# DAIRLab/dair_pll

Measured on NVIDIA B200. Metric: ContactNets loss+backward samples/s, cube fp64, higher is better.
Workload: dtype f64

## Files before the change

dair_pll_b200/csrc/cn_cube.cuh:

```cuda
#pragma once
#include "cn_common.cuh"

#ifndef CN_STAT_LS
#define CN_STAT_LS()
#define CN_STAT_UNIT()
#endif

namespace cn {

constexpr int CUBE_NQ = 7, CUBE_NV = 6, CUBE_NX = 13, CUBE_NC = 4, CUBE_K = 12;
constexpr int CUBE_NPARAM = 14;
constexpr int CUBE_PROB_FIELDS = 33;

template <typename T> struct CubeParams {
  T m, c[3], Isym[6];
  T mu;
  T h[3];
  T dt, eps, inv_eps, grav;
  T Io[6];
  T Isym_inv[6];
  T inv_m;
  T dscale[6];
};

template <typename T>
CN_HD void cube_params_init(CubeParams<T>& P, const T* inertia, const T* mu, const T* half, T dt, T eps) {
  P.m = inertia[0];
  for (int i = 0; i < 3; ++i) P.c[i] = inertia[1 + i];
  for (int i = 0; i < 6; ++i) P.Isym[i] = inertia[4 + i];
  P.mu = mu[0];
  for (int i = 0; i < 3; ++i) P.h[i] = half[i];
  P.dt = dt; P.eps = eps; P.inv_eps = T(1) / eps; P.grav = T(9.81);
  const T cx = P.c[0], cy = P.c[1], cz = P.c[2], m = P.m;
  P.Io[0] = P.Isym[0] + m * (cy * cy + cz * cz);
  P.Io[1] = P.Isym[1] + m * (cx * cx + cz * cz);
  P.Io[2] = P.Isym[2] + m * (cx * cx + cy * cy);
  P.Io[3] = P.Isym[3] - m * cx * cy;
  P.Io[4] = P.Isym[4] - m * cx * cz;
  P.Io[5] = P.Isym[5] - m * cy * cz;
  sym3_inv(P.Isym, P.Isym_inv);
  P.inv_m = T(1) / m;
  P.dscale[0] = T(1) / P.Io[0]; P.dscale[1] = T(1) / P.Io[1]; P.dscale[2] = T(1) / P.Io[2];
  P.dscale[3] = P.dscale[4] = P.dscale[5] = P.inv_m;
}

template <typename T> struct CubeProb {
  T* p;
  int s;
  CN_HD T& IW(int i) const { return p[i * s]; }
  CN_HD T& mcW(int i) const { return p[(6 + i) * s]; }
  CN_HD T& rho(int k) const { return p[(9 + k) * s]; }
  CN_HD T& q(int k) const { return p[(21 + k) * s]; }
};

template <typename T>
CN_HD void cube_minv(const CubeParams<T>& P, const T* R, const T* tau, const T* frc, T* aw, T* av) {
  T fb[3], cxf[3], rhs[3], cxa[3], rc[3];
  rot3t(R, frc, fb);
  cross3(P.c, fb, cxf);
  for (int i = 0; i < 3; ++i) rhs[i] = tau[i] - cxf[i];
  sym3_mul(P.Isym_inv, rhs, aw);
  cross3(P.c, aw, cxa);
  rot3(R, cxa, rc);
  for (int i = 0; i < 3; ++i) av[i] = frc[i] * P.inv_m + rc[i];
}

template <typename T>
CN_HD void cube_mass_mul(const CubeParams<T>& P, const CubeProb<T>& S, const T* u, T* o) {
  const T I0 = S.IW(0), I1 = S.IW(1), I2 = S.IW(2), I3 = S.IW(3), I4 = S.IW(4), I5 = S.IW(5);
  const T mc[3] = {S.mcW(0), S.mcW(1), S.mcW(2)};
  T b[3], c[3];
  cross3(mc, u + 3, b);
  cross3(mc, u, c);
  o[0] = I0 * u[0] + I3 * u[1] + I4 * u[2] + b[0];
  o[1] = I3 * u[0] + I1 * u[1] + I5 * u[2] + b[1];
  o[2] = I4 * u[0] + I5 * u[1] + I2 * u[2] + b[2];
  for (int i = 0; i < 3; ++i) o[3 + i] = P.m * u[3 + i] - c[i];
}

template <typename T> CN_HD uint32_t cube_select_corners(const T* d, const T* h) {
  const T a0 = t_abs(d[0]) * h[0], a1 = t_abs(d[1]) * h[1], a2 = t_abs(d[2]) * h[2];
  const uint32_t best = (d[0] >= T(0) ? 4u : 0u) | (d[1] >= T(0) ? 2u : 0u) | (d[2] >= T(0) ? 1u : 0u);
  const bool c01 = a0 <= a1, c12 = a1 <= a2, c02 = a0 <= a2;
  const int is = c01 ? (c02 ? 0 : 2) : (c12 ? 1 : 2);
  const int il = c01 ? (c12 ? 2 : 1) : (c02 ? 2 : 0);
  const int im = 3 - is - il;
  const T lo01 = t_min(a0, a1), hi01 = t_max(a0, a1);
  const T as = t_min(lo01, a2), al = t_max(hi01, a2), am = t_max(lo01, t_min(hi01, a2));
  const uint32_t bs = 4u >> is, bm = 4u >> im, bl = 4u >> il;
  const uint32_t v3 = (as + am <= al) ? (best ^ bs ^ bm) : (best ^ bl);
  uint32_t mask = (1u << best) | (1u << (best ^ bs)) | (1u << (best ^ bm)) | (1u << v3);
  uint32_t sel = 0;
#pragma unroll
  for (int c = 0; c < 4; ++c) {
#if defined(__CUDA_ARCH__)
    const uint32_t i = (uint32_t)(__ffs((int)mask) - 1);
#else
    const uint32_t i = (uint32_t)(__builtin_ffs((int)mask) - 1);
#endif
    mask &= mask - 1u;
    sel |= i << (3 * c);
  }
  return sel;
}

template <typename T> CN_HD T sgn_bit(uint32_t sel, int c, int axis) {
  return ((sel >> (3 * c + 2 - axis)) & 1u) ? T(1) : T(-1);
}

template <typename T, int UNR>
CN_HD void cube_geometry(const CubeParams<T>& P, const T* quat, T* R, uint32_t& sel, const CubeProb<T>& S) {
  quat_to_rot(quat, R);
  T A[9];
#pragma unroll
  for (int i = 0; i < 3; ++i) {
    const T r0 = R[3 * i], r1 = R[3 * i + 1], r2 = R[3 * i + 2];
    A[3 * i + 0] = r0 * P.Io[0] + r1 * P.Io[3] + r2 * P.Io[4];
    A[3 * i + 1] = r0 * P.Io[3] + r1 * P.Io[1] + r2 * P.Io[5];
    A[3 * i + 2] = r0 * P.Io[4] + r1 * P.Io[5] + r2 * P.Io[2];
  }
  S.IW(0) = A[0] * R[0] + A[1] * R[1] + A[2] * R[2];
  S.IW(1) = A[3] * R[3] + A[4] * R[4] + A[5] * R[5];
  S.IW(2) = A[6] * R[6] + A[7] * R[7] + A[8] * R[8];
  S.IW(3) = A[0] * R[3] + A[1] * R[4] + A[2] * R[5];
  S.IW(4) = A[0] * R[6] + A[1] * R[7] + A[2] * R[8];
  S.IW(5) = A[3] * R[6] + A[4] * R[7] + A[5] * R[8];
  T cW[3];
  rot3(R, P.c, cW);
#pragma unroll
  for (int i = 0; i < 3; ++i) S.mcW(i) = P.m * cW[i];
  const T d[3] = {-R[6], -R[7], -R[8]};
  sel = cube_select_corners(d, P.h);
  T Rh[9];
#pragma unroll
  for (int i = 0; i < 3; ++i)
#pragma unroll
    for (int k = 0; k < 3; ++k) Rh[3 * i + k] = R[3 * i + k] * P.h[k];
#pragma unroll UNR
  for (int c = 0; c < CUBE_NC; ++c) {
    const T sx = sgn_bit<T>(sel, c, 0), sy = sgn_bit<T>(sel, c, 1), sz = sgn_bit<T>(sel, c, 2);
#pragma unroll
    for (int i = 0; i < 3; ++i) S.rho(3 * c + i) = sx * Rh[3 * i] + sy * Rh[3 * i + 1] + sz * Rh[3 * i + 2];
  }
}

template <typename T>
CN_HD void cube_free_accel(const CubeParams<T>& P, const T* R, const T* wB, T* aw, T* av) {
  T Iw[3], wIw[3], gB[3], cg[3], tau[3], wc[3], wwc[3], Rwwc[3], frc[3];
  sym3_mul(P.Io, wB, Iw);
  cross3(wB, Iw, wIw);
  gB[0] = -P.grav * R[6]; gB[1] = -P.grav * R[7]; gB[2] = -P.grav * R[8];
  cross3(P.c, gB, cg);
  for (int i = 0; i < 3; ++i) tau[i] = -wIw[i] + P.m * cg[i];
  cross3(wB, P.c, wc);
  cross3(wB, wc, wwc);
  rot3(R, wwc, Rwwc);
  for (int i = 0; i < 3; ++i) frc[i] = -P.m * Rwwc[i];
  frc[2] -= P.m * P.grav;
  cube_minv(P, R, tau, frc, aw, av);
}

template <typename T>
CN_HD void cube_contact_residual(const CubeParams<T>& P, const CubeProb<T>& S, int c, const T* u, T* rho, T* r) {
  rho[0] = S.rho(3 * c); rho[1] = S.rho(3 * c + 1); rho[2] = S.rho(3 * c + 2);
  T e[3];
  cross3_add(u, rho, u + 3, e);
  r[0] = P.mu * e[0] + S.q(3 * c);
  r[1] = P.mu * e[1] + S.q(3 * c + 1);
  r[2] = e[2] + S.q(3 * c + 2);
}

template <typename T, bool WANT_H, int UNR>
CN_HD void cube_eval(const CubeParams<T>& P, const CubeProb<T>& S, const T* u, T* g, T* H, T& res2, T& scale2) {
  T Mu[6];
  cube_mass_mul(P, S, u, Mu);
  T z[6] = {T(0), T(0), T(0), T(0), T(0), T(0)};
  if (WANT_H) {
    const T m0 = S.mcW(0), m1 = S.mcW(1), m2 = S.mcW(2);
    H[0] = S.IW(0); H[7] = S.IW(1); H[14] = S.IW(2);
    H[6] = S.IW(3); H[12] = S.IW(4); H[13] = S.IW(5);
    H[18] = T(0); H[19] = m2;   H[20] = -m1;
    H[24] = -m2;  H[25] = T(0); H[26] = m0;
    H[30] = m1;   H[31] = -m0;  H[32] = T(0);
    H[21] = P.m; H[28] = P.m; H[35] = P.m; H[27] = T(0); H[33] = T(0); H[34] = T(0);
  }
#pragma unroll UNR
  for (int c = 0; c < CUBE_NC; ++c) {
    T rho[3], r[3], f[3], K[6];
    cube_contact_residual(P, S, c, u, rho, r);
    cone_eval<T, WANT_H>(r, P.inv_eps, P.mu, f, K);
    const T ft[3] = {P.mu * f[0], P.mu * f[1], f[2]};
    cross3_add(rho, ft, z, z);
#pragma unroll
    for (int i = 0; i < 3; ++i) z[3 + i] += ft[i];
    if (WANT_H) {
      const T K0[3] = {K[0], K[1], K[2]}, K1[3] = {K[1], K[3], K[4]}, K2[3] = {K[2], K[4], K[5]};
      T P0[3], P1[3], P2[3];
      cross3(rho, K0, P0); cross3(rho, K1, P1); cross3(rho, K2, P2);
#pragma unroll
      for (int i = 0; i < 3; ++i) { H[18 + i] += P0[i]; H[24 + i] += P1[i]; H[30 + i] += P2[i]; }
      const T a = rho[0], b = rho[1], cz = rho[2];
      H[0] = H[0] + b * P2[0] - cz * P1[0];
      H[6] = H[6] + b * P2[1] - cz * P1[1];
      H[7] = H[7] + cz * P0[1] - a * P2[1];
      H[12] = H[12] + b * P2[2] - cz * P1[2];
      H[13] = H[13] + cz * P0[2] - a * P2[2];
      H[14] = H[14] + a * P1[2] - b * P0[2];
      H[21] += K[0]; H[27] += K[1]; H[28] += K[3]; H[33] += K[2]; H[34] += K[4]; H[35] += K[5];
    }
  }
  res2 = T(0); T a2 = T(0), b2 = T(0);
#pragma unroll
  for (int i = 0; i < 6; ++i) {
    g[i] = Mu[i] - z[i];
    res2 += g[i] * g[i] * P.dscale[i];
    a2 += Mu[i] * Mu[i] * P.dscale[i];
    b2 += z[i] * z[i] * P.dscale[i];
  }
  scale2 = t_max(a2, b2);
}

template <typename T, int UNR> CN_HD bool cube_trivially_solved(const CubeProb<T>& S) {
  bool open = true;
#pragma unroll UNR
  for (int c = 0; c < CUBE_NC; ++c) {
    const T q0 = S.q(3 * c), q1 = S.q(3 * c + 1), qn = S.q(3 * c + 2);
    open = open && (qn >= T(0)) && (q0 * q0 + q1 * q1 <= qn * qn);
  }
  return open;
}

template <typename T> CN_HD bool cube_converged(const SolverCfg<T>& cfg, T res2, T scale2) {
  return !(res2 > cfg.tol_rel * cfg.tol_rel * scale2);
}

enum { NEWTON_DONE = 0, NEWTON_CONTINUE = 1 };

template <typename T> struct CubeTrial {
  T alpha, lo, hi;
};

template <typename T, int UNR>
CN_HD int cube_newton_visit(const CubeParams<T>& P, const CubeProb<T>& S, const SolverCfg<T>& cfg, T* u, T* d,
                            T& d0, T& best_res2, CubeTrial<T>& tr, int& it) {
  T g[6], H[36], res2, scale2;
  CN_STAT_UNIT();
  cube_eval<T, true, UNR>(P, S, u, g, H, res2, scale2);
  if (cube_converged(cfg, res2, scale2)) {
    if (cfg.polish && res2 == res2) {
      block_solve6_neg<T>(H, g, d);
#pragma unroll
      for (int i = 0; i < 6; ++i) u[i] += d[i];
    }
    return NEWTON_DONE;
  }
  if (res2 <= cfg.tol_stall * cfg.tol_stall * scale2 && !(res2 < T(0.25) * best_res2)) {
    it += 1 << 16;
    if ((it >> 16) >= 3) return NEWTON_DONE;
  } else if (res2 < best_res2 || best_res2 < T(0)) {
    it &= 0xffff;
  }
  if (res2 < best_res2 || best_res2 < T(0)) best_res2 = res2;
  const int trials = (it >> 8) & 0xff;
  if (d0 < T(0) && trials != 0xff) {
    T d1 = T(0);
#pragma unroll
    for (int i = 0; i < 6; ++i) d1 += g[i] * d[i];
    const T thresh = -cfg.ls_c * d0;
    const bool accept = trials == 0 ? (d1 <= thresh) : (t_abs(d1) <= thresh);
    if (!accept) {
      if (d1 < T(0)) tr.lo = tr.alpha; else tr.hi = tr.alpha;
      T d2 = T(0);
#pragma unroll
      for (int i = 0; i < 6; ++i) {
        T row = T(0);
#pragma unroll
        for (int j = 0; j < 6; ++j) row += H[j <= i ? 6 * i + j : 6 * j + i] * d[j];
        d2 += d[i] * row;
      }
      T an = tr.alpha - d1 * t_rcp(d2);
      if (!(an > tr.lo && an < tr.hi)) an = T(0.5) * (tr.lo + tr.hi);
      int nt = trials + 1;
      if (tr.hi - tr.lo <= T(4) * eps_of<T>() * tr.hi || nt >= 7) {
        an = tr.lo > T(0) ? tr.lo : an;
        nt = 0xff;
      }
      const T step = an - tr.alpha;
#pragma unroll
      for (int i = 0; i < 6; ++i) u[i] += step * d[i];
      tr.alpha = an;
      it = (it & ~0xff00) | (nt << 8);
      return NEWTON_CONTINUE;
    }
  }
  if ((it & 0xff) >= cfg.max_iter) return NEWTON_DONE;
  block_solve6_neg<T>(H, g, d);
  T dd = T(0);
#pragma unroll
  for (int i = 0; i < 6; ++i) { dd += g[i] * d[i]; u[i] += d[i]; }
  d0 = dd < T(0) ? dd : T(0);
  tr.alpha = T(1); tr.lo = T(0); tr.hi = T(1);
  it = (it & ~0xff00) + 1;
  if (res2 <= cfg.tol_final * cfg.tol_final * scale2) return NEWTON_DONE;
  return NEWTON_CONTINUE;
}

template <typename T, int UNR>
CN_HD int cube_solve(const CubeParams<T>& P, const CubeProb<T>& S, const SolverCfg<T>& cfg, T* u) {
  int it = 0;
  if (cube_trivially_solved<T, UNR>(S)) {
#pragma unroll
    for (int i = 0; i < 6; ++i) u[i] = T(0);
  } else {
    T d[6], d0 = T(0), best = T(-1);
    CubeTrial<T> tr{T(1), T(0), T(1)};
    while (cube_newton_visit<T, UNR>(P, S, cfg, u, d, d0, best, tr, it) != NEWTON_DONE) {}
  }
  return it & 0xff;
}

template <typename T> struct CubeLossAux {
  T R[9];
  T dv[6];
  T acc[6];
  T vp[6];
  T pos_z;
  T konst;
  T dvW[6];
  T a_min;
  uint32_t sel;
};

#ifndef CN_LOSS_START_FACTOR
#define CN_LOSS_START_FACTOR 7.0
#endif

template <typename T, int UNR>
CN_HD void cube_loss_prologue(const CubeParams<T>& P, const T* x, const T* xp, const CubeProb<T>& S,
                              CubeLossAux<T>& A) {
  cube_geometry<T, UNR>(P, xp, A.R, A.sel, S);
  A.pos_z = xp[6];
#pragma unroll
  for (int i = 0; i < 6; ++i) A.vp[i] = xp[7 + i];
  cube_free_accel(P, A.R, A.vp, A.acc, A.acc + 3);
#pragma unroll
  for (int i = 0; i < 6; ++i) A.dv[i] = A.vp[i] - (x[7 + i] + P.dt * A.acc[i]);
  T dvW[6], vW[6];
  rot3(A.R, A.dv, dvW); rot3(A.R, A.vp, vW);
#pragma unroll
  for (int i = 0; i < 3; ++i) { dvW[3 + i] = A.dv[3 + i]; vW[3 + i] = A.vp[3 + i]; }
  T pen4 = T(0), a_min = T(2);
#pragma unroll UNR
  for (int c = 0; c < CUBE_NC; ++c) {
    const T rho[3] = {S.rho(3 * c), S.rho(3 * c + 1), S.rho(3 * c + 2)};
    T ed[3], ev[3];
    cross3_add(dvW, rho, dvW + 3, ed); cross3_add(vW, rho, vW + 3, ev);
    const T sx = P.mu * ev[0], sy = P.mu * ev[1];
    const T speed2 = sx * sx + sy * sy;
    const T speed = speed2 * t_rsqrt0(speed2);
    const T phic = rho[2] + A.pos_z;
    const T s0 = P.dt * sx, s1 = P.dt * sy, s2 = t_abs(phic) + P.dt * speed;
    const T e0 = -P.mu * ed[0], e1 = -P.mu * ed[1], e2 = -ed[2];
    S.q(3 * c) = e0 + s0;
    S.q(3 * c + 1) = e1 + s1;
    S.q(3 * c + 2) = e2 + s2;
    const T pneg2 = t_abs(phic) - phic;
    pen4 += pneg2 * pneg2;
    if (CN_LOSS_START_FACTOR > 0) {
      const T Aq = e0 * e0 + e1 * e1 - e2 * e2, Bh = s0 * e0 + s1 * e1 - s2 * e2;
      const T cs = s0 * s0 + s1 * s1 - s2 * s2;
      const T Cq = T(0.5) * (cs - t_abs(cs));
      const T disc = Bh * Bh - Aq * Cq;
      const T den = Bh + disc * t_rsqrt0(disc);
      const T a_c = den > T(0) ? -Cq * t_rcp(den) : T(2);
      a_min = a_c < a_min ? a_c : a_min;
    }
  }
  const T pen = T(0.25) * pen4;
  A.a_min = a_min;
#pragma unroll
  for (int i = 0; i < 6; ++i) A.dvW[i] = dvW[i];
  T Mdv[6];
  cube_mass_mul(P, S, dvW, Mdv);
  T e = T(0);
#pragma unroll
  for (int i = 0; i < 6; ++i) e += dvW[i] * Mdv[i];
  A.konst = T(0.5) * e + pen;
}

template <typename T> CN_HD void cube_loss_start_fraction(const CubeLossAux<T>& A, T a, T* u) {
#pragma unroll
  for (int i = 0; i < 6; ++i) u[i] = (T(1) - a) * A.dvW[i];
}
template <typename T> CN_HD void cube_loss_start(const CubeLossAux<T>& A, T factor, T* u) {
  cube_loss_start_fraction<T>(A, factor > T(0) ? t_min(factor * A.a_min, T(1)) : T(1), u);
}

template <typename T> CN_HD void vex3(const T* X, T* o) {
  o[0] = X[7] - X[5]; o[1] = X[2] - X[6]; o[2] = X[3] - X[1];
}

template <typename T>
CN_HD void rigid_body_inertia_adjoint(T m, const T* c, const T* R, const T* w, T grav, T* Kww, const T* N, T trvv,
                                      const T* lam, T* grad) {
  T wxl[3];
  cross3(w, lam, wxl);
#pragma unroll
  for (int i = 0; i < 3; ++i)
#pragma unroll
    for (int j = 0; j < 3; ++j) Kww[3 * i + j] += wxl[i] * w[j];
  grad[4] += Kww[0]; grad[5] += Kww[4]; grad[6] += Kww[8];
  grad[7] += Kww[1] + Kww[3]; grad[8] += Kww[2] + Kww[6]; grad[9] += Kww[5] + Kww[7];
  const T trK = Kww[0] + Kww[4] + Kww[8];
  T Kc[3], Ktc[3];
#pragma unroll
  for (int i = 0; i < 3; ++i) {
    Kc[i] = Kww[3 * i] * c[0] + Kww[3 * i + 1] * c[1] + Kww[3 * i + 2] * c[2];
    Ktc[i] = Kww[i] * c[0] + Kww[3 + i] * c[1] + Kww[6 + i] * c[2];
  }
  const T cc = dot3(c, c);
  T NR[9];
#pragma unroll
  for (int i = 0; i < 3; ++i)
#pragma unroll
    for (int j = 0; j < 3; ++j) NR[3 * i + j] = N[3 * i] * R[j] + N[3 * i + 1] * R[3 + j] + N[3 * i + 2] * R[6 + j];
  T vNR[3];
  vex3(NR, vNR);
  const T gB[3] = {-grav * R[6], -grav * R[7], -grav * R[8]};
  T ell[3];
  rot3t(R, lam + 3, ell);
  T cxg[3], wc[3], wwc[3], wl[3], wwl[3], gxl[3];
  cross3(c, gB, cxg);
  cross3(w, c, wc); cross3(w, wc, wwc);
  cross3(w, ell, wl); cross3(w, wl, wwl);
  cross3(gB, lam, gxl);
  grad[0] += cc * trK - dot3(c, Kc) + dot3(c, vNR) + trvv + dot3(lam, cxg) - dot3(ell, wwc) - grav * lam[5];
#pragma unroll
  for (int i = 0; i < 3; ++i)
    grad[1 + i] += m * (T(2) * trK * c[i] - Kc[i] - Ktc[i] + vNR[i] + gxl[i] - wwl[i]);
}

template <typename T, int UNR, bool PARK = false>
CN_HD T cube_loss_epilogue(const CubeParams<T>& P, const CubeProb<T>& S, const CubeLossAux<T>& A, const T* u,
                           T* grad, T* force_out) {
  const T* R = A.R;
  T zW[6] = {T(0), T(0), T(0), T(0), T(0), T(0)};
  T qf = T(0), ff = T(0);
  bool fok = true;
#pragma unroll UNR
  for (int c = 0; c < CUBE_NC; ++c) {
    T rho[3], r[3], f[3];
    cube_contact_residual(P, S, c, u, rho, r);
    cone_eval<T, false>(r, P.inv_eps, P.mu, f, (T*)nullptr);
    const T ft[3] = {P.mu * f[0], P.mu * f[1], f[2]};
    cross3_add(rho, ft, zW, zW);
#pragma unroll
    for (int i = 0; i < 3; ++i) {
      zW[3 + i] += ft[i];
      qf += S.q(3 * c + i) * f[i]; ff += f[i] * f[i];
      fok = fok && t_abs(f[i]) <= T(1e3);
    }
    if (PARK) {
#pragma unroll
      for (int i = 0; i < 3; ++i) S.q(3 * c + i) = f[i];
    }
    if (force_out) { force_out[c] = f[2]; force_out[4 + 2 * c] = f[0]; force_out[4 + 2 * c + 1] = f[1]; }
  }
  if (!fok) {
    if (force_out) for (int i = 0; i < 12; ++i) force_out[i] = T(0);
    return T(0);
  }
  T z[6], y[6];
  rot3t(R, zW, z);
#pragma unroll
  for (int i = 0; i < 3; ++i) z[3 + i] = zW[3 + i];
  cube_minv(P, R, z, z + 3, y, y + 3);
  T zy = T(0);
#pragma unroll
  for (int i = 0; i < 6; ++i) zy += z[i] * y[i];
  const T loss = T(0.5) * zy + T(0.5) * P.eps * ff + qf + A.konst;
  if (!grad) return loss;

  const T* dv = A.dv; const T* a = A.acc; const T* w = A.vp;
  T lam[6], b[6];
#pragma unroll
  for (int i = 0; i < 6; ++i) { b[i] = y[i] - dv[i]; lam[i] = P.dt * b[i]; }
  T Kww[9], N[9], trvv = T(0);
#pragma unroll
  for (int i = 0; i < 3; ++i)
#pragma unroll
    for (int j = 0; j < 3; ++j) {
      Kww[3 * i + j] = T(0.5) * (dv[i] * dv[j] - y[i] * y[j]) - lam[i] * a[j];
      N[3 * i + j] = (dv[i] * dv[3 + j] - y[i] * y[3 + j]) - lam[i] * a[3 + j] - lam[3 + j] * a[i];
    }
#pragma unroll
  for (int i = 0; i < 3; ++i) trvv += T(0.5) * (dv[3 + i] * dv[3 + i] - y[3 + i] * y[3 + i]) - lam[3 + i] * a[3 + i];
  rigid_body_inertia_adjoint<T>(P.m, P.c, R, w, P.grav, Kww, N, trvv, lam, grad);
  T bW[3], wW[3];
  rot3(R, b, bW); rot3(R, w, wW);
  T gmu = T(0), gh0 = T(0), gh1 = T(0), gh2 = T(0);
#pragma unroll UNR
  for (int cidx = 0; cidx < CUBE_NC; ++cidx) {
    T rho[3], r[3], f[3];
    if (PARK) {
#pragma unroll
      for (int i = 0; i < 3; ++i) { rho[i] = S.rho(3 * cidx + i); f[i] = S.q(3 * cidx + i); }
    } else {
      cube_contact_residual(P, S, cidx, u, rho, r);
      cone_eval<T, false>(r, P.inv_eps, P.mu, f, (T*)nullptr);
    }
    T eb[3], ev[3];
    cross3_add(bW, rho, b + 3, eb); cross3_add(wW, rho, A.vp + 3, ev);
    const T ftx = f[0], fty = f[1], fn = f[2];
    const T sx = P.mu * ev[0], sy = P.mu * ev[1];
    const T sinv = t_rsqrt0(sx * sx + sy * sy);
    const T ux = sx * sinv, uy = sy * sinv;
    const T gx = P.dt * (fn * ux + ftx), gy = P.dt * (fn * uy + fty);
    gmu = gmu + ftx * eb[0] + fty * eb[1] + gx * ev[0] + gy * ev[1];
    const T phic = rho[2] + A.pos_z;
    const T phibar = (phic > T(0) ? fn : (phic < T(0) ? -fn : T(0))) - (t_abs(phic) - phic);
    const T ft[3] = {P.mu * ftx, P.mu * fty, fn};
    const T gt[3] = {P.mu * gx, P.mu * gy, T(0)};
    T p[3], pB[3];
    cross3(ft, bW, p);
    cross3_add(gt, wW, p, p);
    p[2] += phibar;
    rot3t(R, p, pB);
    gh0 += sgn_bit<T>(A.sel, cidx, 0) * pB[0];
    gh1 += sgn_bit<T>(A.sel, cidx, 1) * pB[1];
    gh2 += sgn_bit<T>(A.sel, cidx, 2) * pB[2];
  }
  grad[10] += gmu;
  grad[11] += gh0; grad[12] += gh1; grad[13] += gh2;
  return loss;
}

template <typename T>
CN_HD bool cube_loss_free_flight(const CubeParams<T>& P, const T* x, const T* xp, T* grad, T* loss_out) {
  T R[9], vp[6], acc[6], dv[6];
  quat_to_rot(xp, R);
  const T dsup[3] = {-R[6], -R[7], -R[8]};
  const uint32_t sel = cube_select_corners(dsup, P.h);
#pragma unroll
  for (int i = 0; i < 6; ++i) vp[i] = xp[7 + i];
  cube_free_accel(P, R, vp, acc, acc + 3);
#pragma unroll
  for (int i = 0; i < 6; ++i) dv[i] = vp[i] - (x[7 + i] + P.dt * acc[i]);
  T dvW[3], vW[3], Rh[9];
  rot3(R, dv, dvW); rot3(R, vp, vW);
#pragma unroll
  for (int i = 0; i < 3; ++i)
#pragma unroll
    for (int k = 0; k < 3; ++k) Rh[3 * i + k] = R[3 * i + k] * P.h[k];
  bool open = true;
  T pen4 = T(0), gs[3] = {T(0), T(0), T(0)};
#pragma unroll 1
  for (int c = 0; c < CUBE_NC; ++c) {
    const T sx = sgn_bit<T>(sel, c, 0), sy = sgn_bit<T>(sel, c, 1), sz = sgn_bit<T>(sel, c, 2);
    T rho[3], ed[3], ev[3];
#pragma unroll
    for (int i = 0; i < 3; ++i) rho[i] = sx * Rh[3 * i] + sy * Rh[3 * i + 1] + sz * Rh[3 * i + 2];
    cross3_add(dvW, rho, dv + 3, ed); cross3_add(vW, rho, vp + 3, ev);
    const T tx = P.mu * ev[0], ty = P.mu * ev[1];
    const T speed2 = tx * tx + ty * ty;
    const T speed = speed2 * t_rsqrt0(speed2);
    const T phic = rho[2] + xp[6];
    const T q0 = -P.mu * ed[0] + P.dt * tx, q1 = -P.mu * ed[1] + P.dt * ty;
    const T qn = -ed[2] + t_abs(phic) + P.dt * speed;
    open = open && (qn >= T(0)) && (q0 * q0 + q1 * q1 <= qn * qn);
    const T pneg2 = t_abs(phic) - phic;
    pen4 += pneg2 * pneg2;
    gs[0] -= sx * pneg2; gs[1] -= sy * pneg2; gs[2] -= sz * pneg2;
  }
  if (!open) return false;
  const T pen = T(0.25) * pen4;
  const T gh[3] = {gs[0] * R[6], gs[1] * R[7], gs[2] * R[8]};
  T vB[3], Iw[3], cxv[3];
  rot3t(R, dv + 3, vB);
  sym3_mul(P.Io, dv, Iw);
  cross3(P.c, vB, cxv);
  const T e = dot3(dv, Iw) + T(2) * P.m * dot3(dv, cxv) + P.m * dot3(dv + 3, dv + 3);
  *loss_out = T(0.5) * e + pen;
  if (grad) {
    T lam[6], Kww[9], N[9], trvv = T(0);
#pragma unroll
    for (int i = 0; i < 6; ++i) lam[i] = -P.dt * dv[i];
#pragma unroll
    for (int i = 0; i < 3; ++i)
#pragma unroll
      for (int j = 0; j < 3; ++j) {
        Kww[3 * i + j] = T(0.5) * dv[i] * dv[j] - lam[i] * acc[j];
        N[3 * i + j] = dv[i] * dv[3 + j] - lam[i] * acc[3 + j] - lam[3 + j] * acc[i];
      }
#pragma unroll
    for (int i = 0; i < 3; ++i) trvv += T(0.5) * dv[3 + i] * dv[3 + i] - lam[3 + i] * acc[3 + i];
    rigid_body_inertia_adjoint<T>(P.m, P.c, R, vp, P.grav, Kww, N, trvv, lam, grad);
    grad[11] += gh[0]; grad[12] += gh[1]; grad[13] += gh[2];
  }
  return true;
}

template <typename T>
CN_HD T cube_loss_sample(const CubeParams<T>& P, const SolverCfg<T>& cfg, const T* x, const T* xp, T* grad,
                         T* force_out, int* iters_out) {
  T store[CUBE_PROB_FIELDS];
  const CubeProb<T> S{store, 1};
  CubeLossAux<T> A;
  cube_loss_prologue<T, 4>(P, x, xp, S, A);
  T u[6];
  cube_loss_start<T>(A, T(CN_LOSS_START_FACTOR), u);
  const int it = cube_solve<T, 4>(P, S, cfg, u);
  if (iters_out) *iters_out = it;
  return cube_loss_epilogue<T, 4>(P, S, A, u, grad, force_out);
}

template <typename T> struct CubeStepAux {
  T R[9];
  T vm[6];
  uint32_t sel;
};

template <typename T, int UNR>
CN_HD void cube_step_prologue(const CubeParams<T>& P, const T* x, const CubeProb<T>& S, CubeStepAux<T>& A) {
  T acc[6], vmW[6];
  cube_geometry<T, UNR>(P, x, A.R, A.sel, S);
  cube_free_accel(P, A.R, x + 7, acc, acc + 3);
#pragma unroll
  for (int i = 0; i < 6; ++i) A.vm[i] = x[7 + i] + P.dt * acc[i];
  rot3(A.R, A.vm, vmW);
#pragma unroll
  for (int i = 0; i < 3; ++i) vmW[3 + i] = A.vm[3 + i];
  const T inv_dt = T(1) / P.dt;
#pragma unroll UNR
  for (int c = 0; c < CUBE_NC; ++c) {
    const T rho[3] = {S.rho(3 * c), S.rho(3 * c + 1), S.rho(3 * c + 2)};
    T e[3];
    cross3(vmW, rho, e);
    S.q(3 * c) = P.mu * (e[0] + vmW[3]);
    S.q(3 * c + 1) = P.mu * (e[1] + vmW[4]);
    S.q(3 * c + 2) = (e[2] + vmW[5]) + (rho[2] + x[6]) * inv_dt;
  }
}

template <typename T, int UNR>
CN_HD void cube_step_epilogue(const CubeParams<T>& P, const CubeProb<T>& S, const CubeStepAux<T>& A, const T* x,
                              const T* u, T* xn, T* force_out) {
  if (force_out) {
#pragma unroll UNR
    for (int c = 0; c < CUBE_NC; ++c) {
      T rho[3], r[3], f[3];
      cube_contact_residual(P, S, c, u, rho, r);
      cone_eval<T, false>(r, P.inv_eps, P.mu, f, (T*)nullptr);
      force_out[c] = f[2]; force_out[4 + 2 * c] = f[0]; force_out[4 + 2 * c + 1] = f[1];
    }
  }
  T uB[3], vn[6];
  rot3t(A.R, u, uB);
#pragma unroll
  for (int i = 0; i < 3; ++i) { vn[i] = A.vm[i] + uB[i]; vn[3 + i] = A.vm[3 + i] + u[3 + i]; }
  const T rx = vn[0] * P.dt, ry = vn[1] * P.dt, rz = vn[2] * P.dt;
  const T ang = t_sqrt(rx * rx + ry * ry + rz * rz);
  const T half = T(0.5) * ang;
  const T sinc = half > T(0) ? sin(half) / half : T(1);
  const T dw = cos(half), k = T(0.5) * sinc;
  const T dx = rx * k, dy = ry * k, dz = rz * k;
  const T qw = x[0], qx = x[1], qy = x[2], qz = x[3];
  xn[0] = qw * dw - (qx * dx + qy * dy + qz * dz);
  xn[1] = qw * dx + dw * qx + (qy * dz - qz * dy);
  xn[2] = qw * dy + dw * qy + (qz * dx - qx * dz);
  xn[3] = qw * dz + dw * qz + (qx * dy - qy * dx);
#pragma unroll
  for (int i = 0; i < 3; ++i) xn[4 + i] = x[4 + i] + vn[3 + i] * P.dt;
#pragma unroll
  for (int i = 0; i < 6; ++i) xn[7 + i] = vn[i];
}

template <typename T>
CN_HD int cube_step_sample(const CubeParams<T>& P, const SolverCfg<T>& cfg, const T* x, T* xn, T* force_out,
                           T* warm = nullptr) {
  T store[CUBE_PROB_FIELDS];
  const CubeProb<T> S{store, 1};
  CubeStepAux<T> A;
  cube_step_prologue<T, 4>(P, x, S, A);
  T u[6];
#pragma unroll
  for (int i = 0; i < 6; ++i) u[i] = warm ? warm[i] : T(0);
  const int it = cube_solve<T, 4>(P, S, cfg, u);
  cube_step_epilogue<T, 4>(P, S, A, x, u, xn, force_out);
  if (warm) {
#pragma unroll
    for (int i = 0; i < 6; ++i) warm[i] = u[i];
  }
  return it;
}

template <typename T> CN_HD T contact_off() { return T(1e30); }

template <typename T>
CN_HD void body_geometry_pts(const CubeParams<T>& P, const T* quat, const T* pts, int n_c, T* R, const CubeProb<T>& S) {
  quat_to_rot(quat, R);
  T A[9];
#pragma unroll
  for (int i = 0; i < 3; ++i) {
    const T r0 = R[3 * i], r1 = R[3 * i + 1], r2 = R[3 * i + 2];
    A[3 * i + 0] = r0 * P.Io[0] + r1 * P.Io[3] + r2 * P.Io[4];
    A[3 * i + 1] = r0 * P.Io[3] + r1 * P.Io[1] + r2 * P.Io[5];
    A[3 * i + 2] = r0 * P.Io[4] + r1 * P.Io[5] + r2 * P.Io[2];
  }
  S.IW(0) = A[0] * R[0] + A[1] * R[1] + A[2] * R[2];
  S.IW(1) = A[3] * R[3] + A[4] * R[4] + A[5] * R[5];
  S.IW(2) = A[6] * R[6] + A[7] * R[7] + A[8] * R[8];
  S.IW(3) = A[0] * R[3] + A[1] * R[4] + A[2] * R[5];
  S.IW(4) = A[0] * R[6] + A[1] * R[7] + A[2] * R[8];
  S.IW(5) = A[3] * R[6] + A[4] * R[7] + A[5] * R[8];
  T cW[3];
  rot3(R, P.c, cW);
#pragma unroll
  for (int i = 0; i < 3; ++i) S.mcW(i) = P.m * cW[i];
#pragma unroll
  for (int c = 0; c < CUBE_NC; ++c) {
    T r[3] = {T(0), T(0), T(0)};
    if (c < n_c) rot3(R, pts + 3 * c, r);
#pragma unroll
    for (int i = 0; i < 3; ++i) S.rho(3 * c + i) = r[i];
  }
}

template <typename T>
CN_HD T body_loss_sample_pts(const CubeParams<T>& P, const SolverCfg<T>& cfg, const T* x, const T* xp, const T* pts,
                             int n_c, T* grad11, T* grad_pts, T* force_out, int* iters_out) {
  T store[CUBE_PROB_FIELDS];
  const CubeProb<T> S{store, 1};
  T R[9], vp[6], acc[6], dv[6];
  body_geometry_pts(P, xp, pts, n_c, R, S);
  const T pos_z = xp[6];
#pragma unroll
  for (int i = 0; i < 6; ++i) vp[i] = xp[7 + i];
  cube_free_accel(P, R, vp, acc, acc + 3);
#pragma unroll
  for (int i = 0; i < 6; ++i) dv[i] = vp[i] - (x[7 + i] + P.dt * acc[i]);
  T dvW[6], vW[6];
  rot3(R, dv, dvW); rot3(R, vp, vW);
#pragma unroll
  for (int i = 0; i < 3; ++i) { dvW[3 + i] = dv[3 + i]; vW[3 + i] = vp[3 + i]; }
  T pen = T(0);
#pragma unroll
  for (int c = 0; c < CUBE_NC; ++c) {
    if (c < n_c) {
      const T rho[3] = {S.rho(3 * c), S.rho(3 * c + 1), S.rho(3 * c + 2)};
      T ed[3], ev[3];
      cross3(dvW, rho, ed); cross3(vW, rho, ev);
#pragma unroll
      for (int i = 0; i < 3; ++i) { ed[i] += dvW[3 + i]; ev[i] += vW[3 + i]; }
      const T sx = P.mu * ev[0], sy = P.mu * ev[1];
      const T speed2 = sx * sx + sy * sy;
      const T speed = speed2 * t_rsqrt(t_max(speed2, t_tiny<T>()));
      const T phic = rho[2] + pos_z;
      S.q(3 * c) = -P.mu * ed[0] + P.dt * sx;
      S.q(3 * c + 1) = -P.mu * ed[1] + P.dt * sy;
      S.q(3 * c + 2) = -ed[2] + t_abs(phic) + P.dt * speed;
      const T pneg = t_max(-phic, T(0));
      pen += pneg * pneg;
    } else {
      S.q(3 * c) = T(0); S.q(3 * c + 1) = T(0); S.q(3 * c + 2) = contact_off<T>();
    }
// ... 450 lines not shown
```

dair_pll_b200/csrc/cn_kernels.cu:

```cuda
#include <cuda_runtime.h>

#include "../../include/dair_pll_b200.h"
#include "cn_cube.cuh"
#include "cn_params.cuh"
#include "cn_elbow.cuh"
#include "cn_elbow_wf.cuh"
#include "cn_comm.cuh"
#include "cn_launch.cuh"
#include "cn_reduce.cuh"

namespace {

constexpr int kLossThreads = 128;
constexpr int kNAcc = 16;
constexpr int kMaxBlocks = 148 * 16;
static_assert((size_t)kMaxBlocks * kNAcc * sizeof(double) <= cn::kWsPartialsBytes, "box partials exceed the workspace");

inline int rollout_tosses_per_warp(int64_t B, int sms, int64_t resident_warps) {
  const int64_t warps1 = (int64_t)sms * (kLossThreads / 32);
  int64_t lpw = (B + warps1 - 1) / warps1;
  if (lpw > 12) lpw = (B + resident_warps - 1) / resident_warps;
  if (lpw < 1) lpw = 1;
  if (lpw > 32) lpw = 32;
  return (int)lpw;
// ... 152 lines not shown
  int n_act = 0, n_done = kWfSlots, h_act = 0, h_done = 0, n_in = 0, h_in = 0;
  if (race_warp) {
    const int64_t first = ((int64_t)blockIdx.x * kWfWarps + warp) * kRaceSamples;
    const int64_t left = head - first;
    const int cnt = left <= 0 ? 0 : (left < kRaceSamples ? (int)left : kRaceSamples);
    if (lane < cnt * kRaceLanes) pool->q_in[lane] = (int32_t)(first + lane / kRaceLanes) | ((lane % kRaceLanes) << 28);
    n_in = cnt * kRaceLanes;
  }
  __syncwarp();

  while (true) {
    int phase;
    const bool drain = next >= hi && n_in == 0;
    if (next < hi && n_in < 32) phase = 2;
    else if (drain) {
      if (n_act > 0) phase = 1;
      else if (n_done > 0) phase = 0;
      else break;
    } else if (n_done >= kWfPeMin) phase = 0;
    else phase = 1;

    if (phase == 2) {
      int64_t first = next;
      if (dyn_counter) {
        unsigned long long t = 0;
        if (lane == 0) t = atomicAdd(dyn_counter, 32ull);
        first = (int64_t)__shfl_sync(0xffffffffu, t, 0);
        if (first >= B) first = B;
      }
      const int64_t left = hi - first;
      const int cnt = left < 32 ? (int)left : 32;
      bool queue = false;
      const int64_t b = first + lane;
      if (lane < cnt) {
        T xs[13], xps[13];
#pragma unroll
        for (int i = 0; i < 13; ++i) { xs[i] = T(x[b * ldx + i]); xps[i] = T(xp[b * ldxp + i]); }
        T gs[DPLL_CUBE_NPARAM];
#pragma unroll
        for (int i = 0; i < DPLL_CUBE_NPARAM; ++i) gs[i] = T(0);
        T l = T(0);
        if constexpr (PTS) {
          const T w = weight ? T(weight[b]) : T(1);
          if (cn::body_loss_free_flight_pts<T>(P, xs, xps, half + b * 12, want_grad >> 1, w, (want_grad & 1) ? gs : (T*)nullptr,
                                               u_out ? u_out + b * 12 : (IO*)nullptr, &l)) {
            if (force) {
#pragma unroll
              for (int i = 0; i < 12; ++i) force[b * 12 + i] = IO(0);
            }
#pragma unroll
            for (int i = 0; i < 11; ++i) acc[i] += w * gs[i];
            if (loss) loss[b] = IO(l);
            acc[11] += l;
            if (iters) iters[b] = 0;
          } else {
            queue = true;
          }
        } else
        if (cn::cube_loss_free_flight<T>(P, xs, xps, want_grad ? gs : (T*)nullptr, &l)) {
          if (force) {
#pragma unroll
            for (int i = 0; i < 12; ++i) force[b * 12 + i] = IO(0);
          }
          const T w = weight ? T(weight[b]) : T(1);
#pragma unroll
          for (int i = 0; i < DPLL_CUBE_NPARAM; ++i) acc[i] += w * gs[i];
          if (loss) loss[b] = IO(l);
          acc[14] += l;
          if (iters) iters[b] = 0;
          if (u_out) {
#pragma unroll
            for (int i = 0; i < 6; ++i) u_out[b * 6 + i] = IO(0);
          }
        } else {
          queue = true;
        }
      }
      const unsigned m_q = __ballot_sync(0xffffffffu, queue);
      if (queue) pool->q_in[(h_in + n_in + __popc(m_q & lt_mask)) % kWfQin] = (int32_t)(b - lo);
      n_in += __popc(m_q);
      next = dyn_counter ? (first >= B ? B : lo) : next + cnt;
#ifndef CN_NO_PREFETCH
      if (!dyn_counter && next + lane < hi) {
        const char* px = reinterpret_cast<const char*>(x + (next + lane) * ldx);
        const char* pp = reinterpret_cast<const char*>(xp + (next + lane) * ldxp);
        asm volatile("prefetch.global.L2 [%0];" ::"l"(px));
        asm volatile("prefetch.global.L2 [%0];" ::"l"(px + 13 * sizeof(IO) - 1));
        asm volatile("prefetch.global.L2 [%0];" ::"l"(pp));
        asm volatile("prefetch.global.L2 [%0];" ::"l"(pp + 13 * sizeof(IO) - 1));
      }
#endif
    } else if (phase == 1) {
      const int k = n_act < 32 ? n_act : 32;
      const bool on = lane < k;
      int st = -1;
      int slot = 0;
      if (on) {
        slot = pool->q_act[(h_act + lane) % kWfSlots];
        const cn::CubeProb<T> S{&pool->field[0][slot], kWfSlots};
        T u[6], d[6];
#pragma unroll
        for (int i = 0; i < 6; ++i) { u[i] = pool->field[33 + i][slot]; d[i] = pool->field[40 + i][slot]; }
        T best = pool->field[39][slot], d0 = pool->field[46][slot];
        cn::CubeTrial<T> tr{pool->field[47][slot], pool->field[48][slot], pool->field[49][slot]};
        int it = pool->iters[slot];
        st = cn::cube_newton_visit<T, UNR>(P, S, cfg, u, d, d0, best, tr, it);
        pool->iters[slot] = it;
        pool->field[39][slot] = best;
#pragma unroll
        for (int i = 0; i < 6; ++i) { pool->field[33 + i][slot] = u[i]; pool->field[40 + i][slot] = d[i]; }
        pool->field[46][slot] = d0;
        pool->field[47][slot] = tr.alpha; pool->field[48][slot] = tr.lo; pool->field[49][slot] = tr.hi;
      }
      if (race_warp) {
        const int sid = on ? pool->sample[slot] : -2 - lane;
        const unsigned grp = __match_any_sync(0xffffffffu, sid);
        const unsigned fin = __ballot_sync(0xffffffffu, on && st == cn::NEWTON_DONE);
        if (on && (grp & fin) && lane != __ffs(grp & fin) - 1) { pool->sample[slot] = -1; st = cn::NEWTON_DONE; }
      }
      __syncwarp();
      const unsigned m_done = __ballot_sync(0xffffffffu, st == cn::NEWTON_DONE);
      const unsigned m_act = __ballot_sync(0xffffffffu, st == cn::NEWTON_CONTINUE);
      h_act = (h_act + k) % kWfSlots; n_act -= k;
      if (st == cn::NEWTON_DONE) pool->q_done[(h_done + n_done + __popc(m_done & lt_mask)) % kWfSlots] = (uint8_t)slot;
      else if (st == cn::NEWTON_CONTINUE) pool->q_act[(h_act + n_act + __popc(m_act & lt_mask)) % kWfSlots] = (uint8_t)slot;
      n_done += __popc(m_done); n_act += __popc(m_act);
    } else {
      const int k = n_done < 32 ? n_done : 32;
      const bool on = lane < k;
      int slot = 0, old = -1;
      if (on) { slot = pool->q_done[(h_done + lane) % kWfSlots]; old = pool->sample[slot]; }
      bool to_active = false;
      int n_new = 0;
#pragma unroll 1
      for (int pass = 0; pass < 2; ++pass) {
        if (pass == 0) {
          if (!__any_sync(0xffffffffu, on && old >= 0)) continue;
        } else {
          n_new = n_in < k ? n_in : k;
          if (n_new == 0) break;
        }
        const bool work = pass == 0 ? (on && old >= 0) : (lane < n_new);
        if (work) {
          const int32_t ent = pass == 0 ? old : pool->q_in[(h_in + lane) % kWfQin];
          const int start = race_warp ? (ent >> 28) & 7 : 0;
          const int64_t b = lo + (race_warp ? (ent & 0x0fffffff) : ent);
          T xs[13], xps[13];
#pragma unroll
          for (int i = 0; i < 13; ++i) { xs[i] = T(x[b * ldx + i]); xps[i] = T(xp[b * ldxp + i]); }
          const cn::CubeProb<T> S{&pool->field[0][slot], kWfSlots};
          cn::CubeLossAux<T> A;
          if constexpr (PTS) cn::body_loss_prologue_pts<T, kWfUnrPE>(P, xs, xps, half + b * 12, want_grad >> 1, S, A);
          else
          cn::cube_loss_prologue<T, kWfUnrPE>(P, xs, xps, S, A);
          if (pass == 0) {
            if constexpr (PTS) {
              T u[6], gs[11], fo[12];
#pragma unroll
              for (int i = 0; i < 6; ++i) u[i] = pool->field[33 + i][slot];
#pragma unroll
              for (int i = 0; i < 11; ++i) gs[i] = T(0);
              const T w = weight ? T(weight[b]) : T(1);
              const T l = cn::body_loss_epilogue_pts<T, kWfUnrPE, true>(P, S, A, u, want_grad >> 1, w,
                                                                        (want_grad & 1) ? gs : (T*)nullptr,
                                                                        u_out ? u_out + b * 12 : (IO*)nullptr,
                                                                        force ? fo : (T*)nullptr);
              if (force) {
#pragma unroll
                for (int i = 0; i < 12; ++i) force[b * 12 + i] = IO(fo[i]);
              }
#pragma unroll
              for (int i = 0; i < 11; ++i) acc[i] += w * gs[i];
              if (loss) loss[b] = IO(l);
              acc[11] += l;
              if (iters) iters[b] = pool->iters[slot] & 0xff;
            } else {
            T u[6];
#pragma unroll
            for (int i = 0; i < 6; ++i) u[i] = pool->field[33 + i][slot];
            T gs[DPLL_CUBE_NPARAM];
#pragma unroll
            for (int i = 0; i < DPLL_CUBE_NPARAM; ++i) gs[i] = T(0);
            T fo[12];
            const T l = cn::cube_loss_epilogue<T, kWfUnrPE, true>(P, S, A, u, want_grad ? gs : (T*)nullptr, force ? fo : (T*)nullptr);
            if (force) {
#pragma unroll
              for (int i = 0; i < 12; ++i) force[b * 12 + i] = IO(fo[i]);
            }
            const T w = weight ? T(weight[b]) : T(1);
#pragma unroll
            for (int i = 0; i < DPLL_CUBE_NPARAM; ++i) acc[i] += w * gs[i];
            if (loss) loss[b] = IO(l);
            acc[14] += l;
            if (iters) iters[b] = pool->iters[slot] & 0xff;
            if (u_out) {
#pragma unroll
              for (int i = 0; i < 6; ++i) u_out[b * 6 + i] = IO(u[i]);
            }
            }
            pool->sample[slot] = -1;
          } else {
            T us[6];
            if (start == 3) cn::cube_loss_start_fraction<T>(A, T(0.3), us);
            else cn::cube_loss_start<T>(A, start == 1 ? T(2) : start == 2 ? T(60) : T(CN_LOSS_START_FACTOR), us);
#pragma unroll
            for (int i = 0; i < 6; ++i) pool->field[33 + i][slot] = u_init ? T(u_init[b * 6 + i]) : us[i];
            pool->field[39][slot] = T(-1);
            pool->field[46][slot] = T(0);
            pool->sample[slot] = (int32_t)(b - lo);
            pool->iters[slot] = 0;
            to_active = true;
          }
        }
      }
      h_in = (h_in + n_new) % kWfQin; n_in -= n_new;
      const bool more = next < hi || n_in > 0;
      __syncwarp();
      const unsigned m_act = __ballot_sync(0xffffffffu, to_active);
      const unsigned m_keep = __ballot_sync(0xffffffffu, on && !to_active && more);
      h_done = (h_done + k) % kWfSlots; n_done -= k;
      if (to_active) pool->q_act[(h_act + n_act + __popc(m_act & lt_mask)) % kWfSlots] = (uint8_t)slot;
      else if (on && more) pool->q_done[(h_done + n_done + __popc(m_keep & lt_mask)) % kWfSlots] = (uint8_t)slot;
      n_act += __popc(m_act); n_done += __popc(m_keep);
    }
    __syncwarp();
  }

  if (!partials) return;
  __shared__ T red[kWfWarps][kNAcc];
#pragma unroll 1
  for (int i = 0; i < kNAcc; ++i) {
    T v = T(0);
#pragma unroll
    for (int j = 0; j < kNAcc; ++j) v = (j == i) ? acc[j] : v;
    const T s = warp_sum(v);
    if (lane == 0) red[warp][i] = s;
  }
  __syncthreads();
  if (threadIdx.x < kNAcc) {
    T s = T(0);
#pragma unroll
    for (int w = 0; w < kWfWarps; ++w) s += red[w][threadIdx.x];
    partials[(int64_t)blockIdx.x * kNAcc + threadIdx.x] = s;
  }
}


template <typename T, typename IO>
__global__ void cube_prep_kernel(const IO* __restrict__ theta, const IO* __restrict__ friction,
                                 const IO* __restrict__ length, IO* __restrict__ params ,
                                 const int32_t* __restrict__ skip_flag) {
  if (skip_flag && *skip_flag) return;
  if (threadIdx.x == 0) {
    T th[10], out[10];
    for (int i = 0; i < 10; ++i) th[i] = T(theta[i]);
    cn::theta_to_inertia_vector<T>(th, out);
    for (int i = 0; i < 10; ++i) params[i] = IO(out[i]);
    const T a = cn::t_abs(T(friction[0])), b = cn::t_abs(T(friction[1]));
    params[10] = IO(T(2) * a * b / (a + b));
    for (int i = 0; i < 3; ++i) params[11 + i] = IO(cn::t_abs(T(length[i])));
  }
}

template <typename T, typename IO>
__global__ void reduce_partials_leaf_kernel(const T* __restrict__ partials, int nblocks, const IO* __restrict__ theta,
                                            const IO* __restrict__ friction, const IO* __restrict__ length,
                                            IO* __restrict__ grad_leaf, IO* __restrict__ loss_sum,
                                            const int32_t* __restrict__ skip_flag, cn::CommDev* comm, double count,
                                            IO* __restrict__ sums, IO* __restrict__ means, IO* __restrict__ local_out) {
  if (skip_flag && *skip_flag) return;
  __shared__ T g[kNAcc];
  __shared__ double o[cn::COMM_MAX_ELEMS];
  const int lane = threadIdx.x & 31, w = threadIdx.x >> 5;
  if (w < kNAcc) {
    T s = T(0);
    for (int b = lane; b < nblocks; b += 32) s += partials[(int64_t)b * kNAcc + w];
    s = warp_sum(s);
    if (lane == 0) g[w] = s;
  }
  __syncthreads();
  const int t = threadIdx.x;
  if (t < 10) {
    cn::Dual<T> th[10], out[10];
    for (int i = 0; i < 10; ++i) th[i] = cn::Dual<T>(T(theta[i]), i == t ? T(1) : T(0));
    cn::theta_to_inertia_vector<cn::Dual<T>>(th, out);
    T s = T(0);
    for (int i = 0; i < 10; ++i) s += g[i] * out[i].d;
    o[t] = (double)s;
  } else if (t == 10) {
    const T fa = T(friction[0]), fb = T(friction[1]);
    const T a = cn::t_abs(fa), b = cn::t_abs(fb), den = (a + b) * (a + b);
    const T sa = fa > T(0) ? T(1) : (fa < T(0) ? T(-1) : T(0)), sb = fb > T(0) ? T(1) : (fb < T(0) ? T(-1) : T(0));
    o[10] = (double)(g[10] * (T(2) * b * b / den) * sa);
    o[11] = (double)(g[10] * (T(2) * a * a / den) * sb);
  } else if (t >= 11 && t < 14) {
    const T l = T(length[t - 11]);
    o[12 + (t - 11)] = (double)(g[t] * (l > T(0) ? T(1) : (l < T(0) ? T(-1) : T(0))));
  } else if (t == 14) {
    o[15] = (double)g[14];
  } else if (t == 15) {
    o[16] = count;
  }
  __syncthreads();
  if (local_out && t < 16) local_out[t] = IO(o[t]);
  if (comm) cn::comm_allreduce_block(comm, o, 17);
  if (t < 15 && grad_leaf) grad_leaf[t] = IO(o[t]);
  else if (t == 15 && loss_sum) *loss_sum = IO(o[15]);
  if (sums && t < 17) sums[t] = IO(o[t]);
  if (means && t < 16) means[t] = IO(o[t] / o[16]);
}

template <typename T, typename IO>
__global__ void __launch_bounds__(kLossThreads)
cube_rollout_kernel(const IO* __restrict__ x0, const IO* __restrict__ inertia, const IO* __restrict__ mu,
                    const IO* __restrict__ half, T dt, T eps, int64_t B, int steps, IO* __restrict__ traj,
                    IO* __restrict__ force, int32_t* __restrict__ iters, int lanes_per_warp, IO* __restrict__ usol) {
  const int lane = threadIdx.x & 31;
  if (lane >= lanes_per_warp) return;
  cn::CubeParams<T> P;
  load_cube_params<T, IO>(P, inertia, mu, half, dt, eps);
  const cn::SolverCfg<T> cfg = cn::default_cfg<T>();
  const int64_t warp = ((int64_t)blockIdx.x * blockDim.x + threadIdx.x) >> 5;
  const int64_t stride = (((int64_t)gridDim.x * blockDim.x) >> 5) * lanes_per_warp;
  for (int64_t b = warp * lanes_per_warp + lane; b < B; b += stride) {
    T xc[13], xn[13], fo[12];
    IO* out = traj + b * (int64_t)(steps + 1) * 13;
#pragma unroll
    for (int i = 0; i < 13; ++i) { xc[i] = T(x0[b * 13 + i]); out[i] = IO(xc[i]); }
    int total = 0;
    T warm[6] = {T(0), T(0), T(0), T(0), T(0), T(0)};
    for (int s = 0; s < steps; ++s) {
      total += cn::cube_step_sample<T>(P, cfg, xc, xn, force ? fo : nullptr, warm);
      if (usol) {
#pragma unroll
        for (int i = 0; i < 6; ++i) usol[(b * steps + s) * 6 + i] = IO(warm[i]);
      }
      if (force) {
#pragma unroll
        for (int i = 0; i < 12; ++i) force[(b * steps + s) * 12 + i] = IO(fo[i]);
      }
#pragma unroll
      for (int i = 0; i < 13; ++i) { xc[i] = xn[i]; out[(int64_t)(s + 1) * 13 + i] = IO(xn[i]); }
    }
    if (iters) iters[b] = total;
  }
}

template <typename T, typename IO>
__global__ void __launch_bounds__(kLossThreads)
body_pts_step_kernel(const IO* __restrict__ x, const IO* __restrict__ inertia, const IO* __restrict__ mu,
                     const IO* __restrict__ pts, int n_c, T dt, T eps, int64_t B, IO* __restrict__ xn,
                     IO* __restrict__ force) {
  cn::CubeParams<T> P;
  {
// ... 455 lines not shown
```

Baseline: 3.228 billion.

## Split cube loss prologue into state, build and finalise phases per pass

The cube loss prologue is split into three phases. A cheap state phase computes rotation, corner selection and velocity deltas. A build phase writes slot geometry and cone data and runs only when a sample is first admitted. A finalise phase computes penalty and mass energy from the stored slot fields and runs only at retirement. This avoids recomputing slot geometry and the cone setup on both passes of the wavefront kernel, and the free-flight check now returns early at the first closed contact. The risk is that finalise reads slot fields written during build, so it depends on the slot geometry being unchanged while the solve runs.

```diff
diff --git a/dair_pll_b200/csrc/cn_cube.cuh b/dair_pll_b200/csrc/cn_cube.cuh
--- a/dair_pll_b200/csrc/cn_cube.cuh
+++ b/dair_pll_b200/csrc/cn_cube.cuh
@@ -108,9 +108,13 @@
   return ((sel >> (3 * c + 2 - axis)) & 1u) ? T(1) : T(-1);
 }
 
+template <typename T> CN_HD uint32_t cube_contact_corners(const CubeParams<T>& P, const T* R) {
+  const T d[3] = {-R[6], -R[7], -R[8]};
+  return cube_select_corners(d, P.h);
+}
+
 template <typename T, int UNR>
-CN_HD void cube_geometry(const CubeParams<T>& P, const T* quat, T* R, uint32_t& sel, const CubeProb<T>& S) {
-  quat_to_rot(quat, R);
+CN_HD void cube_slot_geometry(const CubeParams<T>& P, const T* R, uint32_t sel, const CubeProb<T>& S) {
   T A[9];
 #pragma unroll
   for (int i = 0; i < 3; ++i) {
@@ -129,8 +133,6 @@
   rot3(R, P.c, cW);
 #pragma unroll
   for (int i = 0; i < 3; ++i) S.mcW(i) = P.m * cW[i];
-  const T d[3] = {-R[6], -R[7], -R[8]};
-  sel = cube_select_corners(d, P.h);
   T Rh[9];
 #pragma unroll
   for (int i = 0; i < 3; ++i)
@@ -142,6 +144,13 @@
 #pragma unroll
     for (int i = 0; i < 3; ++i) S.rho(3 * c + i) = sx * Rh[3 * i] + sy * Rh[3 * i + 1] + sz * Rh[3 * i + 2];
   }
+}
+
+template <typename T, int UNR>
+CN_HD void cube_geometry(const CubeParams<T>& P, const T* quat, T* R, uint32_t& sel, const CubeProb<T>& S) {
+  quat_to_rot(quat, R);
+  sel = cube_contact_corners(P, R);
+  cube_slot_geometry<T, UNR>(P, R, sel, S);
 }
 
 template <typename T>
@@ -335,21 +344,32 @@
 #define CN_LOSS_START_FACTOR 7.0
 #endif
 
-template <typename T, int UNR>
-CN_HD void cube_loss_prologue(const CubeParams<T>& P, const T* x, const T* xp, const CubeProb<T>& S,
-                              CubeLossAux<T>& A) {
-  cube_geometry<T, UNR>(P, xp, A.R, A.sel, S);
+template <typename T> CN_HD void cube_world_twist(const T* R, const T* s, T* o) {
+  rot3(R, s, o);
+#pragma unroll
+  for (int i = 0; i < 3; ++i) o[3 + i] = s[3 + i];
+}
+
+template <typename T>
+CN_HD void cube_loss_state(const CubeParams<T>& P, const T* x, const T* xp, CubeLossAux<T>& A) {
+  quat_to_rot(xp, A.R);
+  A.sel = cube_contact_corners(P, A.R);
   A.pos_z = xp[6];
 #pragma unroll
   for (int i = 0; i < 6; ++i) A.vp[i] = xp[7 + i];
   cube_free_accel(P, A.R, A.vp, A.acc, A.acc + 3);
 #pragma unroll
   for (int i = 0; i < 6; ++i) A.dv[i] = A.vp[i] - (x[7 + i] + P.dt * A.acc[i]);
-  T dvW[6], vW[6];
-  rot3(A.R, A.dv, dvW); rot3(A.R, A.vp, vW);
-#pragma unroll
-  for (int i = 0; i < 3; ++i) { dvW[3 + i] = A.dv[3 + i]; vW[3 + i] = A.vp[3 + i]; }
-  T pen4 = T(0), a_min = T(2);
+  cube_world_twist(A.R, A.dv, A.dvW);
+}
+
+template <typename T, int UNR>
+CN_HD void cube_loss_build(const CubeParams<T>& P, const CubeProb<T>& S, CubeLossAux<T>& A) {
+  cube_slot_geometry<T, UNR>(P, A.R, A.sel, S);
+  const T* dvW = A.dvW;
+  T vW[6];
+  cube_world_twist(A.R, A.vp, vW);
+  T a_min = T(2);
 #pragma unroll UNR
   for (int c = 0; c < CUBE_NC; ++c) {
     const T rho[3] = {S.rho(3 * c), S.rho(3 * c + 1), S.rho(3 * c + 2)};
@@ -364,8 +384,6 @@
     S.q(3 * c) = e0 + s0;
     S.q(3 * c + 1) = e1 + s1;
     S.q(3 * c + 2) = e2 + s2;
-    const T pneg2 = t_abs(phic) - phic;
-    pen4 += pneg2 * pneg2;
     if (CN_LOSS_START_FACTOR > 0) {
       const T Aq = e0 * e0 + e1 * e1 - e2 * e2, Bh = s0 * e0 + s1 * e1 - s2 * e2;
       const T cs = s0 * s0 + s1 * s1 - s2 * s2;
@@ -376,15 +394,24 @@
       a_min = a_c < a_min ? a_c : a_min;
     }
   }
+  A.a_min = a_min;
+}
+
+template <typename T, int UNR>
+CN_HD void cube_loss_finalise(const CubeParams<T>& P, const CubeProb<T>& S, CubeLossAux<T>& A) {
+  T pen4 = T(0);
+#pragma unroll UNR
+  for (int c = 0; c < CUBE_NC; ++c) {
+    const T phic = S.rho(3 * c + 2) + A.pos_z;
+    const T pneg2 = t_abs(phic) - phic;
+    pen4 += pneg2 * pneg2;
+  }
   const T pen = T(0.25) * pen4;
-  A.a_min = a_min;
-#pragma unroll
-  for (int i = 0; i < 6; ++i) A.dvW[i] = dvW[i];
   T Mdv[6];
-  cube_mass_mul(P, S, dvW, Mdv);
+  cube_mass_mul(P, S, A.dvW, Mdv);
   T e = T(0);
 #pragma unroll
-  for (int i = 0; i < 6; ++i) e += dvW[i] * Mdv[i];
+  for (int i = 0; i < 6; ++i) e += A.dvW[i] * Mdv[i];
   A.konst = T(0.5) * e + pen;
 }
 
@@ -552,7 +579,6 @@
   for (int i = 0; i < 3; ++i)
 #pragma unroll
     for (int k = 0; k < 3; ++k) Rh[3 * i + k] = R[3 * i + k] * P.h[k];
-  bool open = true;
   T pen4 = T(0), gs[3] = {T(0), T(0), T(0)};
 #pragma unroll 1
   for (int c = 0; c < CUBE_NC; ++c) {
@@ -567,12 +593,11 @@
     const T phic = rho[2] + xp[6];
     const T q0 = -P.mu * ed[0] + P.dt * tx, q1 = -P.mu * ed[1] + P.dt * ty;
     const T qn = -ed[2] + t_abs(phic) + P.dt * speed;
-    open = open && (qn >= T(0)) && (q0 * q0 + q1 * q1 <= qn * qn);
+    if (!((qn >= T(0)) && (q0 * q0 + q1 * q1 <= qn * qn))) return false;
     const T pneg2 = t_abs(phic) - phic;
     pen4 += pneg2 * pneg2;
     gs[0] -= sx * pneg2; gs[1] -= sy * pneg2; gs[2] -= sz * pneg2;
   }
-  if (!open) return false;
   const T pen = T(0.25) * pen4;
   const T gh[3] = {gs[0] * R[6], gs[1] * R[7], gs[2] * R[8]};
   T vB[3], Iw[3], cxv[3];
@@ -606,11 +631,13 @@
   T store[CUBE_PROB_FIELDS];
   const CubeProb<T> S{store, 1};
   CubeLossAux<T> A;
-  cube_loss_prologue<T, 4>(P, x, xp, S, A);
+  cube_loss_state<T>(P, x, xp, A);
+  cube_loss_build<T, 4>(P, S, A);
   T u[6];
   cube_loss_start<T>(A, T(CN_LOSS_START_FACTOR), u);
   const int it = cube_solve<T, 4>(P, S, cfg, u);
   if (iters_out) *iters_out = it;
+  cube_loss_finalise<T, 4>(P, S, A);
   return cube_loss_epilogue<T, 4>(P, S, A, u, grad, force_out);
 }
 
diff --git a/dair_pll_b200/csrc/cn_kernels.cu b/dair_pll_b200/csrc/cn_kernels.cu
--- a/dair_pll_b200/csrc/cn_kernels.cu
+++ b/dair_pll_b200/csrc/cn_kernels.cu
@@ -328,8 +328,9 @@
           cn::CubeLossAux<T> A;
           if constexpr (PTS) cn::body_loss_prologue_pts<T, kWfUnrPE>(P, xs, xps, half + b * 12, want_grad >> 1, S, A);
           else
-          cn::cube_loss_prologue<T, kWfUnrPE>(P, xs, xps, S, A);
+          cn::cube_loss_state<T>(P, xs, xps, A);
           if (pass == 0) {
+            if constexpr (!PTS) cn::cube_loss_finalise<T, kWfUnrPE>(P, S, A);
             if constexpr (PTS) {
               T u[6], gs[11], fo[12];
 #pragma unroll
@@ -376,6 +377,7 @@
             }
             pool->sample[slot] = -1;
           } else {
+            if constexpr (!PTS) cn::cube_loss_build<T, kWfUnrPE>(P, S, A);
             T us[6];
             if (start == 3) cn::cube_loss_start_fraction<T>(A, T(0.3), us);
             else cn::cube_loss_start<T>(A, start == 1 ? T(2) : start == 2 ? T(60) : T(CN_LOSS_START_FACTOR), us);
```

New measurement: 3.279 billion (median of 6 runs). 1.02x the previous value.
